# microsoft/XPretrain

Measured on NVIDIA H100. Metric: video-text pairs/sec (12f x 224^2, 32 tok), CLIP-ViP ViT-B/16 fwd+InfoNCE+bwd, higher is better.
Workload: dtype bf16

## Files before the change

### xpretrain_b200/csrc/gemm.cu

```cuda
#include "../../include/xpretrain_b200.h"
#include "common.h"
#include "ptx.cuh"
#include <cstdlib>

namespace xp {

constexpr int BM = 128;
constexpr int BK = 64;
constexpr int MMA_K = 16;
constexpr int GEMM_THREADS = 384;

struct GemmDev {
  void* c;
  const float* bias;
  const __nv_bfloat16* residual;
  __nv_bfloat16* aux;
  int M, N, K;
  long long ldc, ldr, ld_aux;
  long long c_group, c_group_stride, r_group, r_group_stride;
  int act;
  int splits;
  int scale_cols;
  float alpha, col_scale;
  uint32_t mn_lbo, mn_sbo;
};

template <int BN>
struct GemmCfg {
  static constexpr int A_BYTES = BM * BK * 2;
  static constexpr int B_BYTES = BN * BK * 2;
  static constexpr int STAGE_BYTES = A_BYTES + B_BYTES;
  static constexpr int STAGES = (BN == 256) ? 4 : 6;
  static constexpr int SMEM_BYTES = STAGES * STAGE_BYTES + 1024 + 256;
};

__device__ __forceinline__ float act_gelu_erf(float x) { return 0.5f * x * (1.f + erff(x * 0.70710678118654752f)); }
__device__ __forceinline__ float act_gelu_erf_grad(float x) {
  float cdf = 0.5f * (1.f + erff(x * 0.70710678118654752f));
  float pdf = 0.3989422804014327f * __expf(-0.5f * x * x);
  return cdf + x * pdf;
}

template <int BN, int A_MN, int B_MN, int OUT, int ACT>
__global__ void __launch_bounds__(GEMM_THREADS, 1)
gemm_kernel(const __grid_constant__ CUtensorMap tmA, const __grid_constant__ CUtensorMap tmB, const GemmDev p) {
  using Cfg = GemmCfg<BN>;
  constexpr int STAGES = Cfg::STAGES;
  constexpr bool PINGPONG = BN == 128;
  constexpr int MH = PINGPONG ? 2 : 1;
  constexpr int NH = BN / 128;
  extern __shared__ uint8_t smem_raw[];
  const uint32_t raw_addr = smem_u32(smem_raw);
  uint8_t* smem = smem_raw + (((raw_addr + 1023u) & ~1023u) - raw_addr);
  uint64_t* full_bar = reinterpret_cast<uint64_t*>(smem + STAGES * Cfg::STAGE_BYTES);
  uint64_t* empty_bar = full_bar + STAGES;

  const int wg = threadIdx.x >> 7;
  const int lane = threadIdx.x & 31;

  const int num_m = (p.M + BM - 1) / BM;
  const int num_n = (p.N + BN - 1) / BN;
  const int num_mn = num_m * num_n;
  const int total = num_mn * p.splits;
  const int kb_total = (p.K + BK - 1) / BK;
  const int kb_per = (kb_total + p.splits - 1) / p.splits;

  if (threadIdx.x == 0) {
    tma_prefetch_desc(&tmA);
    tma_prefetch_desc(&tmB);
    for (int s = 0; s < STAGES; ++s) {
      mbar_init(&full_bar[s], 1);
      mbar_init(&empty_bar[s], PINGPONG ? 1 : 2);
    }
    fence_barrier_init();
  }
  __syncthreads();

  if (wg == 0) {
    setmaxnreg_dec<40>();
    if (threadIdx.x == 0) {
      int stage = 0;
      uint32_t phase = 0;
      for (int tile = blockIdx.x; tile < total; tile += gridDim.x) {
        const int split = tile / num_mn;
        const int mn = tile - split * num_mn;
        const int m_blk = mn / num_n;
        const int n_blk = mn - m_blk * num_n;
        const int k0 = split * kb_per;
        const int k1 = min(kb_total, k0 + kb_per);
        for (int kb = k0; kb < k1; ++kb) {
          mbar_wait_nocall(&empty_bar[stage], phase ^ 1);
          uint8_t* sA = smem + stage * Cfg::STAGE_BYTES;
          uint8_t* sB = sA + Cfg::A_BYTES;
          mbar_arrive_expect_tx(&full_bar[stage], Cfg::STAGE_BYTES);
          if (A_MN) {
#pragma unroll
            for (int i = 0; i < BM / 64; ++i)
              tma_load_2d(sA + i * (BK * 128), &tmA, &full_bar[stage], m_blk * BM + i * 64, kb * BK);
          } else {
            tma_load_2d(sA, &tmA, &full_bar[stage], kb * BK, m_blk * BM);
          }
          if (B_MN) {
#pragma unroll
            for (int i = 0; i < BN / 64; ++i)
              tma_load_2d(sB + i * (BK * 128), &tmB, &full_bar[stage], n_blk * BN + i * 64, kb * BK);
          } else {
            tma_load_2d(sB, &tmB, &full_bar[stage], kb * BK, n_blk * BN);
          }
          if (++stage == STAGES) {
            stage = 0;
            phase ^= 1;
          }
        }
      }
    }
  } else {
    setmaxnreg_inc<232>();
    const int cw = wg - 1;
    const int wq = (threadIdx.x >> 5) & 3;
    constexpr int act = ACT;
    const int N = p.N, scale_cols = p.scale_cols;
    const float alpha = p.alpha, col_scale = p.col_scale;
    __nv_bfloat16* const aux_p = p.aux;
    constexpr bool need_aux_in = (ACT == XP_ACT_DQUICK_GELU || ACT == XP_ACT_DGELU_ERF);
    const __nv_bfloat16* const xin_p = need_aux_in ? p.aux : p.residual;
    constexpr uint32_t A_OFF = 64 * 128;
    const int cta_tiles = (total - blockIdx.x + gridDim.x - 1) / gridDim.x;
    int stage = 0;
    uint32_t phase = 0;
    int local = 0;
    for (int tile = blockIdx.x; tile < total; tile += gridDim.x, ++local) {
      const int split = tile / num_mn;
      const int mn = tile - split * num_mn;
      const int m_blk = mn / num_n;
      const int n_blk = mn - m_blk * num_n;
      const int k0 = split * kb_per;
      const int k1 = min(kb_total, k0 + kb_per);
      if (PINGPONG && (local & 1) != cw) {
        const int next = stage + max(0, k1 - k0);
        phase ^= (next / STAGES) & 1;
        stage = next % STAGES;
        continue;
      }
      if (PINGPONG && local > 0) named_bar_sync(1 + cw, 256);
      const bool pass_turn = PINGPONG && local + 1 < cta_tiles;
      if (k0 >= k1) {
        if (pass_turn) named_bar_arrive(2 - cw, 256);
        continue;
      }
      float acc[MH * NH][64];
#pragma unroll
      for (int q = 0; q < MH * NH; ++q)
#pragma unroll
        for (int i = 0; i < 64; ++i) acc[q][i] = 0.f;
      int prev_stage = -1;
      for (int kb = k0; kb < k1; ++kb) {
        mbar_wait_nocall(&full_bar[stage], phase);
        const uint32_t sA = smem_u32(smem + stage * Cfg::STAGE_BYTES) + (PINGPONG ? 0 : cw * A_OFF);
        const uint32_t sB = smem_u32(smem + stage * Cfg::STAGE_BYTES) + Cfg::A_BYTES;
#pragma unroll
        for (int q = 0; q < MH * NH; ++q) wgmma_fence_regs(acc[q]);
        wgmma_fence();
#pragma unroll
        for (int j = 0; j < BK / MMA_K; ++j) {
#pragma unroll
          for (int mh = 0; mh < MH; ++mh) {
            const uint32_t am = sA + mh * A_OFF;
            const uint64_t adesc = A_MN ? make_smem_desc_sw128(am + j * (MMA_K * 128), p.mn_lbo, p.mn_sbo)
                                        : make_smem_desc_sw128(am + j * (MMA_K * 2), 16, 1024);
#pragma unroll
            for (int h = 0; h < NH; ++h) {
              const uint32_t bh = sB + h * (128 * 128);
              const uint64_t bdesc = B_MN ? make_smem_desc_sw128(bh + j * (MMA_K * 128), p.mn_lbo, p.mn_sbo)
                                          : make_smem_desc_sw128(bh + j * (MMA_K * 2), 16, 1024);
              wgmma_m64n128k16_bf16<A_MN, B_MN>(acc[mh * NH + h], adesc, bdesc);
            }
          }
        }
        wgmma_commit();
#pragma unroll
        for (int q = 0; q < MH * NH; ++q) wgmma_fence_regs(acc[q]);
        wgmma_wait<1>();
        if (prev_stage >= 0 && (threadIdx.x & 127) == 0) mbar_arrive(&empty_bar[prev_stage]);
        prev_stage = stage;
        if (++stage == STAGES) {
          stage = 0;
          phase ^= 1;
        }
      }
      if (pass_turn) named_bar_arrive(2 - cw, 256);
      const auto load_bias = [&](float2(&b)[16], int h) {
#pragma unroll
        for (int i = 0; i < 16; ++i) {
          const int n = n_blk * BN + h * 128 + i * 8 + (lane & 3) * 2;
          b[i] = make_float2(0.f, 0.f);
          if (p.bias != nullptr && split == 0 && n < N) b[i] = __ldg(reinterpret_cast<const float2*>(p.bias + n));
        }
      };
      constexpr bool bias_once = PINGPONG && !need_aux_in;
      float2 bias_tile[16];
      if (bias_once) load_bias(bias_tile, 0);
      wgmma_wait<0>();
#pragma unroll
      for (int q = 0; q < MH * NH; ++q) wgmma_fence_regs(acc[q]);
      if ((threadIdx.x & 127) == 0) mbar_arrive(&empty_bar[prev_stage]);

      const auto apply = [&](float& v0, float& v1, int n, uint32_t xg) -> uint32_t {
        if (n < scale_cols) {
          v0 *= col_scale;
          v1 *= col_scale;
        }
        uint32_t pre = 0;
        if (act == XP_ACT_QUICK_GELU) {
          pre = pack_bf16(v0, v1);
          v0 = quick_gelu(v0);
          v1 = quick_gelu(v1);
        } else if (act == XP_ACT_DQUICK_GELU) {
          v0 *= quick_gelu_grad(bf16_lo(xg));
          v1 *= quick_gelu_grad(bf16_hi(xg));
        } else if (act == XP_ACT_GELU_ERF) {
          pre = pack_bf16(v0, v1);
          v0 = act_gelu_erf(v0);
          v1 = act_gelu_erf(v1);
        } else if (act == XP_ACT_DGELU_ERF) {
          v0 *= act_gelu_erf_grad(bf16_lo(xg));
          v1 *= act_gelu_erf_grad(bf16_hi(xg));
        } else if (xin_p != nullptr) {
          v0 += bf16_lo(xg);
          v1 += bf16_hi(xg);
        }
        return pre;
      };
      constexpr bool save_pre = (ACT == XP_ACT_QUICK_GELU || ACT == XP_ACT_GELU_ERF);
      const int quad = lane & 3;
#pragma unroll
      for (int mh = 0; mh < MH; ++mh) {
        const int row_base = m_blk * BM + (PINGPONG ? mh : cw) * 64 + wq * 16 + (lane >> 2);
#pragma unroll
        for (int rr = 0; rr < 2; ++rr) {
          const int row = row_base + rr * 8;
          const bool row_ok = row < p.M;
          const long long c_off = p.c_group > 0 ? (row / p.c_group) * p.c_group_stride + (row % p.c_group) * p.ldc
                                                : static_cast<long long>(row) * p.ldc;
          const long long x_off = need_aux_in ? static_cast<long long>(row) * p.ld_aux
                                              : (p.r_group > 0 ? (row / p.r_group) * p.r_group_stride + (row % p.r_group) * p.ldr
                                                               : static_cast<long long>(row) * p.ldr);
          const long long a_off = static_cast<long long>(row) * p.ld_aux;
#pragma unroll
          for (int h = 0; h < NH; ++h) {
            const float* const a = acc[mh * NH + h];
            const int n_h = n_blk * BN + h * 128;
            float2 bias2[16];
            if (bias_once) {
#pragma unroll
              for (int i = 0; i < 16; ++i) bias2[i] = bias_tile[i];
            } else {
              load_bias(bias2, h);
            }
            if (OUT == XP_OUT_BF16) {
              uint32_t xin[4][4];
#pragma unroll
              for (int k = 0; k < 4; ++k) {
                const int n8 = n_h + (4 * k + quad) * 8;
                uint4 v = make_uint4(0u, 0u, 0u, 0u);
                if (xin_p != nullptr && row_ok && n8 < N) v = *reinterpret_cast<const uint4*>(xin_p + x_off + n8);
                xin[k][0] = v.x;
                xin[k][1] = v.y;
                xin[k][2] = v.z;
                xin[k][3] = v.w;
                if (xin_p != nullptr) quad_transpose(xin[k]);
              }
#pragma unroll
              for (int k = 0; k < 4; ++k) {
                uint32_t out[4], pre[4];
#pragma unroll
                for (int j = 0; j < 4; ++j) {
                  const int i = 4 * k + j;
                  float v0 = fmaf(a[4 * i + 2 * rr], alpha, bias2[i].x);
                  float v1 = fmaf(a[4 * i + 2 * rr + 1], alpha, bias2[i].y);
                  pre[j] = apply(v0, v1, n_h + i * 8 + quad * 2, xin[k][j]);
                  out[j] = pack_bf16(v0, v1);
                }
                const int n8 = n_h + (4 * k + quad) * 8;
                quad_transpose(out);
                if (row_ok && n8 < N)
                  *reinterpret_cast<uint4*>(static_cast<__nv_bfloat16*>(p.c) + c_off + n8) =
                      make_uint4(out[0], out[1], out[2], out[3]);
                if (save_pre && aux_p != nullptr) {
                  quad_transpose(pre);
                  if (row_ok && n8 < N)
                    *reinterpret_cast<uint4*>(aux_p + a_off + n8) = make_uint4(pre[0], pre[1], pre[2], pre[3]);
                }
              }
            } else if (row_ok) {
              uint32_t xin[16];
#pragma unroll
              for (int i = 0; i < 16; ++i) {
                const int n = n_h + i * 8 + quad * 2;
                xin[i] = 0;
                if (xin_p != nullptr && n < N) xin[i] = *reinterpret_cast<const uint32_t*>(xin_p + x_off + n);
              }
#pragma unroll
              for (int i = 0; i < 16; ++i) {
                const int n = n_h + i * 8 + quad * 2;
                if (n >= N) continue;
                float v0 = fmaf(a[4 * i + 2 * rr], alpha, bias2[i].x);
                float v1 = fmaf(a[4 * i + 2 * rr + 1], alpha, bias2[i].y);
                apply(v0, v1, n, xin[i]);
                if (OUT == XP_OUT_F32) {
                  *reinterpret_cast<float2*>(static_cast<float*>(p.c) + c_off + n) = make_float2(v0, v1);
                } else {
                  asm volatile("red.global.add.v2.f32 [%0], {%1, %2};" ::"l"(static_cast<float*>(p.c) + c_off + n),
                               "f"(v0), "f"(v1)
                               : "memory");
                }
              }
            }
          }
        }
      }
    }
  }
}

template <int BN, int A_MN, int B_MN, int OUT, int ACT>
static int launch_gemm(const CUtensorMap& tmA, const CUtensorMap& tmB, const GemmDev& dev, int grid, cudaStream_t stream) {
  using Cfg = GemmCfg<BN>;
  auto kern = gemm_kernel<BN, A_MN, B_MN, OUT, ACT>;
  static bool attr_set = false;
  if (!attr_set) {
    XP_CHECK_CUDA(cudaFuncSetAttribute(kern, cudaFuncAttributeMaxDynamicSharedMemorySize, Cfg::SMEM_BYTES));
    attr_set = true;
  }
  kern<<<grid, GEMM_THREADS, Cfg::SMEM_BYTES, stream>>>(tmA, tmB, dev);
  XP_CHECK_LAUNCH("gemm_kernel");
  return 0;
}

template <int BN, int OUT, int ACT>
static int dispatch_layout(const XpGemm* g, const CUtensorMap& tmA, const CUtensorMap& tmB, const GemmDev& dev,
                           int grid, cudaStream_t stream) {
  if (g->a_layout == 0 && g->b_layout == 0) return launch_gemm<BN, 0, 0, OUT, ACT>(tmA, tmB, dev, grid, stream);
  if (g->a_layout == 0 && g->b_layout == 1) return launch_gemm<BN, 0, 1, OUT, ACT>(tmA, tmB, dev, grid, stream);
  if (g->a_layout == 1 && g->b_layout == 1) return launch_gemm<BN, 1, 1, OUT, ACT>(tmA, tmB, dev, grid, stream);
  if (g->a_layout == 1 && g->b_layout == 0) return launch_gemm<BN, 1, 0, OUT, ACT>(tmA, tmB, dev, grid, stream);
  return fail("xp_gemm: a_layout/b_layout must be 0 or 1");
}

template <int BN>
static int dispatch_act_bf16(const XpGemm* g, const CUtensorMap& tmA, const CUtensorMap& tmB, const GemmDev& dev, int grid,
                             cudaStream_t stream) {
  switch (g->act) {
    case XP_ACT_NONE: return dispatch_layout<BN, XP_OUT_BF16, XP_ACT_NONE>(g, tmA, tmB, dev, grid, stream);
    case XP_ACT_QUICK_GELU: return dispatch_layout<BN, XP_OUT_BF16, XP_ACT_QUICK_GELU>(g, tmA, tmB, dev, grid, stream);
    case XP_ACT_DQUICK_GELU: return dispatch_layout<BN, XP_OUT_BF16, XP_ACT_DQUICK_GELU>(g, tmA, tmB, dev, grid, stream);
    case XP_ACT_GELU_ERF: return dispatch_layout<BN, XP_OUT_BF16, XP_ACT_GELU_ERF>(g, tmA, tmB, dev, grid, stream);
    case XP_ACT_DGELU_ERF: return dispatch_layout<BN, XP_OUT_BF16, XP_ACT_DGELU_ERF>(g, tmA, tmB, dev, grid, stream);
  }
  return fail("xp_gemm: bad act");
}

template <int BN>
static int dispatch_out(const XpGemm* g, const CUtensorMap& tmA, const CUtensorMap& tmB, const GemmDev& dev, int grid,
                        cudaStream_t stream) {
  switch (g->out) {
    case XP_OUT_BF16: return dispatch_act_bf16<BN>(g, tmA, tmB, dev, grid, stream);
    case XP_OUT_F32: return dispatch_layout<BN, XP_OUT_F32, XP_ACT_NONE>(g, tmA, tmB, dev, grid, stream);
    case XP_OUT_F32_ATOMIC: return dispatch_layout<BN, XP_OUT_F32_ATOMIC, XP_ACT_NONE>(g, tmA, tmB, dev, grid, stream);
  }
  return fail("xp_gemm: bad out mode");
}

static int g_dbg_mn_lbo = 0, g_dbg_mn_sbo = 0;
}

extern "C" void xp_debug_gemm_mn_desc(int lbo, int sbo) {
  xp::g_dbg_mn_lbo = lbo;
  xp::g_dbg_mn_sbo = sbo;
}

extern "C" int xp_gemm(const XpGemm* g, void* stream_v) {
  using namespace xp;
  if (!g) return fail("xp_gemm: null args");
  cudaStream_t stream = static_cast<cudaStream_t>(stream_v);
  if (g->M <= 0 || g->N <= 0 || g->K <= 0) return fail("xp_gemm: M, N, K must be positive");
  if (g->N % 8 != 0) return fail("xp_gemm: N must be a multiple of 8");
  if (!g->a || !g->b || !g->c) return fail("xp_gemm: null operand");
  XP_ENTER(g->a);
  const int splits = g->splits <= 0 ? 1 : g->splits;
  if (splits > 1 && g->out != XP_OUT_F32_ATOMIC) return fail("xp_gemm: split-K requires XP_OUT_F32_ATOMIC");
  if ((g->act == XP_ACT_DQUICK_GELU || g->act == XP_ACT_DGELU_ERF) && !g->aux)
    return fail("xp_gemm: dGELU epilogue needs aux (the forward pre-activation)");
  if (g->act != XP_ACT_NONE && g->out != XP_OUT_BF16) return fail("xp_gemm: activation epilogues need a bf16 output");
  if (g->act != XP_ACT_NONE && g->residual)
    return fail("xp_gemm: a residual add cannot be combined with an activation epilogue");
  if (g->aux && g->c_group > 0) return fail("xp_gemm: aux cannot be combined with grouped rows (c_group > 0)");
  if (g->scale_cols < 0 || g->scale_cols % 2) return fail("xp_gemm: scale_cols must be even and non-negative");
  const int elem_c = g->out == XP_OUT_BF16 ? 2 : 4;
  if ((reinterpret_cast<uintptr_t>(g->c) & 15) || (g->ldc * elem_c) % 16)
    return fail("xp_gemm: C must be 16-byte aligned with a 16-byte multiple row pitch");
  if (g->bias && (reinterpret_cast<uintptr_t>(g->bias) & 15)) return fail("xp_gemm: bias must be 16-byte aligned");
  if (g->residual && ((reinterpret_cast<uintptr_t>(g->residual) & 15) || (g->ldr % 8)))
    return fail("xp_gemm: residual must be 16-byte aligned, ldr % 8 == 0");
  if (g->aux && ((reinterpret_cast<uintptr_t>(g->aux) & 15) || (g->ld_aux % 8)))
    return fail("xp_gemm: aux must be 16-byte aligned, ld_aux % 8 == 0");
  if ((g->c_group > 0 && g->c_group_stride % 8) || (g->r_group > 0 && g->r_group_stride % 8))
    return fail("xp_gemm: c_group_stride / r_group_stride must be multiples of 8 elements");

  const int nsm = sm_count();
  const int num_m = static_cast<int>((g->M + BM - 1) / BM);
  int bn = g->block_n;
  if (bn == 0) {
    const long long tiles256 = static_cast<long long>(num_m) * ((g->N + 255) / 256) * splits;
    const long long kb_split = ((g->K + BK - 1) / BK + splits - 1) / splits;
    const bool short_k_fwd = g->b_layout == 0 && kb_split <= 16;
    bn = (g->N >= 256 && tiles256 >= nsm && !short_k_fwd) ? 256 : 128;
  }
  if (bn != 128 && bn != 256) return fail("xp_gemm: block_n must be 0, 128 or 256");
  if (g->cta_pair < 0 || g->cta_pair > 1) return fail("xp_gemm: cta_pair must be 0 or 1 (no CTA pairs on sm_90)");
  const long long total = static_cast<long long>(num_m) * ((g->N + bn - 1) / bn) * splits;
  int grid = g->max_ctas > 0 ? g->max_ctas : nsm;
  if (grid < 1) grid = 1;
  if (grid > total) grid = static_cast<int>(total);

  CUtensorMap tmA, tmB;
  int rc;
  if (g->a_layout == 0)
    rc = make_tmap_bf16_2d(&tmA, g->a, g->K, g->M, g->lda, BK, BM);
  else
    rc = make_tmap_bf16_2d(&tmA, g->a, g->M, g->K, g->lda, 64, BK);
  if (rc) return rc;
  if (g->b_layout == 0)
    rc = make_tmap_bf16_2d(&tmB, g->b, g->K, g->N, g->ldb, BK, bn);
  else
    rc = make_tmap_bf16_2d(&tmB, g->b, g->N, g->K, g->ldb, 64, BK);
  if (rc) return rc;

  GemmDev dev;
  dev.c = g->c;
  dev.bias = g->bias;
  dev.residual = static_cast<const __nv_bfloat16*>(g->residual);
  dev.aux = static_cast<__nv_bfloat16*>(g->aux);
  dev.M = static_cast<int>(g->M);
  dev.N = static_cast<int>(g->N);
  dev.K = static_cast<int>(g->K);
  dev.ldc = g->ldc;
  dev.ldr = g->ldr;
  dev.ld_aux = g->ld_aux;
  dev.c_group = g->c_group;
  dev.c_group_stride = g->c_group_stride;
  dev.r_group = g->r_group;
  dev.r_group_stride = g->r_group_stride;
  dev.act = g->act;
  dev.splits = splits;
  dev.scale_cols = g->scale_cols;
  dev.alpha = g->alpha;
  dev.col_scale = g->col_scale;
  dev.mn_lbo = g_dbg_mn_lbo ? g_dbg_mn_lbo : BK * 128;
  dev.mn_sbo = g_dbg_mn_sbo ? g_dbg_mn_sbo : 1024;

  return bn == 256 ? dispatch_out<256>(g, tmA, tmB, dev, grid, stream)
                   : dispatch_out<128>(g, tmA, tmB, dev, grid, stream);
}
```

### xpretrain_b200/csrc/ptx.cuh

```cuda
#pragma once
#include <cuda.h>
#include <cuda_bf16.h>
#include <cuda_runtime.h>
#include <stdint.h>
#include <stdio.h>

namespace xp {

#ifndef XP_WAIT_TIMEOUT_CYCLES
#define XP_WAIT_TIMEOUT_CYCLES (8000000000ll)
#endif

__device__ __forceinline__ uint32_t smem_u32(const void* p) {
  return static_cast<uint32_t>(__cvta_generic_to_shared(p));
}
__device__ __forceinline__ int lane_id() { return threadIdx.x & 31; }

__device__ __forceinline__ void mbar_init(uint64_t* bar, uint32_t count) {
  asm volatile("mbarrier.init.shared::cta.b64 [%0], %1;" ::"r"(smem_u32(bar)), "r"(count) : "memory");
}
__device__ __forceinline__ void fence_barrier_init() {
  asm volatile("fence.mbarrier_init.release.cluster;" ::: "memory");
}
__device__ __forceinline__ void fence_proxy_async_smem() {
  asm volatile("fence.proxy.async.shared::cta;" ::: "memory");
}
__device__ __forceinline__ void mbar_arrive_expect_tx(uint64_t* bar, uint32_t bytes) {
  asm volatile("mbarrier.arrive.expect_tx.shared::cta.b64 _, [%0], %1;" ::"r"(smem_u32(bar)), "r"(bytes)
               : "memory");
}
__device__ __forceinline__ void mbar_arrive(uint64_t* bar) {
  asm volatile("mbarrier.arrive.shared::cta.b64 _, [%0];" ::"r"(smem_u32(bar)) : "memory");
}
__device__ __forceinline__ bool mbar_try_wait(uint64_t* bar, uint32_t parity) {
  uint32_t ok;
  asm volatile(
      "{\n"
      ".reg .pred p;\n"
      "mbarrier.try_wait.parity.shared::cta.b64 p, [%1], %2;\n"
      "selp.u32 %0, 1, 0, p;\n"
      "}\n"
      : "=r"(ok)
      : "r"(smem_u32(bar)), "r"(parity)
      : "memory");
  return ok != 0;
}
__device__ __forceinline__ void mbar_wait(uint64_t* bar, uint32_t parity) {
  if (mbar_try_wait(bar, parity)) return;
  long long t0 = clock64();
  while (!mbar_try_wait(bar, parity)) {
    if (clock64() - t0 > XP_WAIT_TIMEOUT_CYCLES) {
      printf("xpretrain_b200: mbarrier wait timeout (block %d thread %d parity %u)\n", blockIdx.x, threadIdx.x,
             parity);
      __trap();
    }
  }
}
__device__ __forceinline__ void mbar_wait_nocall(uint64_t* bar, uint32_t parity) {
  if (mbar_try_wait(bar, parity)) return;
  long long t0 = clock64();
  while (!mbar_try_wait(bar, parity)) {
    if (clock64() - t0 > XP_WAIT_TIMEOUT_CYCLES) __trap();
  }
}

__device__ __forceinline__ void tma_prefetch_desc(const CUtensorMap* m) {
  asm volatile("prefetch.tensormap [%0];" ::"l"(reinterpret_cast<uint64_t>(m)) : "memory");
}
__device__ __forceinline__ void tma_load_2d(void* smem_dst, const CUtensorMap* m, uint64_t* bar, int c0, int c1) {
  asm volatile(
      "cp.async.bulk.tensor.2d.shared::cluster.global.mbarrier::complete_tx::bytes [%0], [%1, {%3, %4}], [%2];"
      ::"r"(smem_u32(smem_dst)), "l"(reinterpret_cast<uint64_t>(m)), "r"(smem_u32(bar)), "r"(c0), "r"(c1)
      : "memory");
}
__device__ __forceinline__ void tma_load_3d(void* smem_dst, const CUtensorMap* m, uint64_t* bar, int c0, int c1,
                                            int c2) {
  asm volatile(
      "cp.async.bulk.tensor.3d.shared::cluster.global.mbarrier::complete_tx::bytes [%0], [%1, {%3, %4, %5}], [%2];"
      ::"r"(smem_u32(smem_dst)), "l"(reinterpret_cast<uint64_t>(m)), "r"(smem_u32(bar)), "r"(c0), "r"(c1), "r"(c2)
      : "memory");
}

__device__ __forceinline__ void tma_store_2d(const CUtensorMap* m, uint32_t smem_src, int c0, int c1) {
  asm volatile("cp.async.bulk.tensor.2d.global.shared::cta.bulk_group [%0, {%2, %3}], [%1];" ::"l"(
                   reinterpret_cast<uint64_t>(m)),
               "r"(smem_src), "r"(c0), "r"(c1)
               : "memory");
}
__device__ __forceinline__ void tma_store_commit() { asm volatile("cp.async.bulk.commit_group;" ::: "memory"); }
template <int N>
__device__ __forceinline__ void tma_store_wait_read() {
  asm volatile("cp.async.bulk.wait_group.read %0;" ::"n"(N) : "memory");
}

__device__ __forceinline__ void wgmma_fence() { asm volatile("wgmma.fence.sync.aligned;" ::: "memory"); }
__device__ __forceinline__ void wgmma_commit() { asm volatile("wgmma.commit_group.sync.aligned;" ::: "memory"); }
template <int N>
__device__ __forceinline__ void wgmma_wait() {
  asm volatile("wgmma.wait_group.sync.aligned %0;" ::"n"(N) : "memory");
}
template <int R>
__device__ __forceinline__ void wgmma_fence_regs(float (&d)[R]) {
#pragma unroll
  for (int i = 0; i < R; ++i) asm volatile("" : "+f"(d[i])::"memory");
}

template <int TA, int TB>
__device__ __forceinline__ void wgmma_m64n128k16_bf16(float (&d)[64], uint64_t adesc, uint64_t bdesc) {
  asm volatile(
      "wgmma.mma_async.sync.aligned.m64n128k16.f32.bf16.bf16 {"
      "%0, %1, %2, %3, %4, %5, %6, %7, %8, %9, %10, %11, %12, %13, %14, %15, "
      "%16, %17, %18, %19, %20, %21, %22, %23, %24, %25, %26, %27, %28, %29, %30, %31, "
      "%32, %33, %34, %35, %36, %37, %38, %39, %40, %41, %42, %43, %44, %45, %46, %47, "
      "%48, %49, %50, %51, %52, %53, %54, %55, %56, %57, %58, %59, %60, %61, %62, %63"
      "}, %64, %65, 1, 1, 1, %66, %67;"
      : "+f"(d[0]), "+f"(d[1]), "+f"(d[2]), "+f"(d[3]), "+f"(d[4]), "+f"(d[5]), "+f"(d[6]), "+f"(d[7]),
        "+f"(d[8]), "+f"(d[9]), "+f"(d[10]), "+f"(d[11]), "+f"(d[12]), "+f"(d[13]), "+f"(d[14]), "+f"(d[15]),
        "+f"(d[16]), "+f"(d[17]), "+f"(d[18]), "+f"(d[19]), "+f"(d[20]), "+f"(d[21]), "+f"(d[22]), "+f"(d[23]),
        "+f"(d[24]), "+f"(d[25]), "+f"(d[26]), "+f"(d[27]), "+f"(d[28]), "+f"(d[29]), "+f"(d[30]), "+f"(d[31]),
        "+f"(d[32]), "+f"(d[33]), "+f"(d[34]), "+f"(d[35]), "+f"(d[36]), "+f"(d[37]), "+f"(d[38]), "+f"(d[39]),
        "+f"(d[40]), "+f"(d[41]), "+f"(d[42]), "+f"(d[43]), "+f"(d[44]), "+f"(d[45]), "+f"(d[46]), "+f"(d[47]),
        "+f"(d[48]), "+f"(d[49]), "+f"(d[50]), "+f"(d[51]), "+f"(d[52]), "+f"(d[53]), "+f"(d[54]), "+f"(d[55]),
        "+f"(d[56]), "+f"(d[57]), "+f"(d[58]), "+f"(d[59]), "+f"(d[60]), "+f"(d[61]), "+f"(d[62]), "+f"(d[63])
      : "l"(adesc), "l"(bdesc), "n"(TA), "n"(TB));
}

template <int TA, int TB>
__device__ __forceinline__ void wgmma_m64n64k16_ss(float (&d)[32], uint64_t adesc, uint64_t bdesc) {
  asm volatile(
      "wgmma.mma_async.sync.aligned.m64n64k16.f32.bf16.bf16 {"
      "%0, %1, %2, %3, %4, %5, %6, %7, %8, %9, %10, %11, %12, %13, %14, %15, "
      "%16, %17, %18, %19, %20, %21, %22, %23, %24, %25, %26, %27, %28, %29, %30, %31"
      "}, %32, %33, 1, 1, 1, %34, %35;"
      : "+f"(d[0]), "+f"(d[1]), "+f"(d[2]), "+f"(d[3]), "+f"(d[4]), "+f"(d[5]), "+f"(d[6]), "+f"(d[7]),
        "+f"(d[8]), "+f"(d[9]), "+f"(d[10]), "+f"(d[11]), "+f"(d[12]), "+f"(d[13]), "+f"(d[14]), "+f"(d[15]),
        "+f"(d[16]), "+f"(d[17]), "+f"(d[18]), "+f"(d[19]), "+f"(d[20]), "+f"(d[21]), "+f"(d[22]), "+f"(d[23]),
        "+f"(d[24]), "+f"(d[25]), "+f"(d[26]), "+f"(d[27]), "+f"(d[28]), "+f"(d[29]), "+f"(d[30]), "+f"(d[31])
      : "l"(adesc), "l"(bdesc), "n"(TA), "n"(TB));
}
template <int TB>
__device__ __forceinline__ void wgmma_m64n64k16_rs(float (&d)[32], const uint32_t (&a)[4], uint64_t bdesc) {
  asm volatile(
      "wgmma.mma_async.sync.aligned.m64n64k16.f32.bf16.bf16 {"
      "%0, %1, %2, %3, %4, %5, %6, %7, %8, %9, %10, %11, %12, %13, %14, %15, "
      "%16, %17, %18, %19, %20, %21, %22, %23, %24, %25, %26, %27, %28, %29, %30, %31"
      "}, {%32, %33, %34, %35}, %36, 1, 1, 1, %37;"
      : "+f"(d[0]), "+f"(d[1]), "+f"(d[2]), "+f"(d[3]), "+f"(d[4]), "+f"(d[5]), "+f"(d[6]), "+f"(d[7]),
        "+f"(d[8]), "+f"(d[9]), "+f"(d[10]), "+f"(d[11]), "+f"(d[12]), "+f"(d[13]), "+f"(d[14]), "+f"(d[15]),
        "+f"(d[16]), "+f"(d[17]), "+f"(d[18]), "+f"(d[19]), "+f"(d[20]), "+f"(d[21]), "+f"(d[22]), "+f"(d[23]),
        "+f"(d[24]), "+f"(d[25]), "+f"(d[26]), "+f"(d[27]), "+f"(d[28]), "+f"(d[29]), "+f"(d[30]), "+f"(d[31])
      : "r"(a[0]), "r"(a[1]), "r"(a[2]), "r"(a[3]), "l"(bdesc), "n"(TB));
}

template <uint32_t N>
__device__ __forceinline__ void setmaxnreg_dec() {
  asm volatile("setmaxnreg.dec.sync.aligned.u32 %0;" ::"n"(N));
}
template <uint32_t N>
__device__ __forceinline__ void setmaxnreg_inc() {
  asm volatile("setmaxnreg.inc.sync.aligned.u32 %0;" ::"n"(N));
}
__device__ __forceinline__ void named_bar_sync(uint32_t id, uint32_t threads) {
  asm volatile("bar.sync %0, %1;" ::"r"(id), "r"(threads) : "memory");
}
__device__ __forceinline__ void named_bar_arrive(uint32_t id, uint32_t threads) {
  asm volatile("bar.arrive %0, %1;" ::"r"(id), "r"(threads) : "memory");
}

__device__ __forceinline__ uint64_t make_smem_desc_sw128(uint32_t smem_addr, uint32_t lbo_bytes,
                                                         uint32_t sbo_bytes) {
  uint64_t d = 0;
  d |= static_cast<uint64_t>((smem_addr & 0x3FFFF) >> 4);
  d |= static_cast<uint64_t>((lbo_bytes >> 4) & 0x3FFF) << 16;
  d |= static_cast<uint64_t>((sbo_bytes >> 4) & 0x3FFF) << 32;
  d |= static_cast<uint64_t>(1) << 62;
  return d;
}

__device__ __forceinline__ void quad_transpose(uint32_t (&v)[4]) {
  const int q = threadIdx.x & 3;
  uint32_t out[4];
  out[0] = out[1] = out[2] = out[3] = 0u;
#pragma unroll
  for (int t = 0; t < 4; ++t) {
    const int j = q ^ t;
    const uint32_t send = j == 0 ? v[0] : j == 1 ? v[1] : j == 2 ? v[2] : v[3];
    const uint32_t got = t == 0 ? send : __shfl_xor_sync(0xffffffffu, send, t);
#pragma unroll
    for (int c = 0; c < 4; ++c)
      if (c == j) out[c] = got;
  }
#pragma unroll
  for (int c = 0; c < 4; ++c) v[c] = out[c];
}

__device__ __forceinline__ uint32_t pack_bf16(float lo, float hi) {
  __nv_bfloat162 v = __floats2bfloat162_rn(lo, hi);
  return *reinterpret_cast<uint32_t*>(&v);
}
__device__ __forceinline__ float bf16_lo(uint32_t v) { return __uint_as_float(v << 16); }
__device__ __forceinline__ float bf16_hi(uint32_t v) { return __uint_as_float(v & 0xFFFF0000u); }

__device__ __forceinline__ float fast_sigmoid(float y) {
  float t;
  asm("tanh.approx.f32 %0, %1;" : "=f"(t) : "f"(0.5f * y));
  return fmaf(0.5f, t, 0.5f);
}
__device__ __forceinline__ float quick_gelu(float x) { return x * fast_sigmoid(1.702f * x); }
__device__ __forceinline__ float quick_gelu_grad(float x) {
  float y = 1.702f * x;
  y = y > 64.f ? 64.f : (y < -64.f ? -64.f : y);
  const float s = fast_sigmoid(y);
  return s * fmaf(y, 1.f - s, 1.f);
}

}
```

Measured before the change: 291.6.

## Stage bf16 GEMM epilogue in swizzled smem and write via TMA stores

For BN=128 ping-pong bf16 GEMMs, each consumer warpgroup now writes its output tile into swizzled shared-memory slots and issues TMA 2D stores instead of per-thread global stores. For dGELU backward it also prefetches the saved pre-activation tile into shared memory via TMA ahead of the epilogue, and it tracks aliasing between input and output. Pipeline stages drop from 6 to 5 to make room for staging buffers. The BN=256 heuristic now treats short-K problems as short regardless of B layout. This adds barrier and store-wait synchronisation and fewer mainloop stages.

```diff
diff --git a/xpretrain_b200/csrc/gemm.cu b/xpretrain_b200/csrc/gemm.cu
--- a/xpretrain_b200/csrc/gemm.cu
+++ b/xpretrain_b200/csrc/gemm.cu
@@ -2,6 +2,7 @@
 #include "common.h"
 #include "ptx.cuh"
 #include <cstdlib>
+#include <cstring>
 
 namespace xp {
 
@@ -23,15 +24,19 @@
   int scale_cols;
   float alpha, col_scale;
   uint32_t mn_lbo, mn_sbo;
+  int xin_alias;
 };
 
-template <int BN>
+template <int BN, bool TMA_OUT>
 struct GemmCfg {
   static constexpr int A_BYTES = BM * BK * 2;
   static constexpr int B_BYTES = BN * BK * 2;
   static constexpr int STAGE_BYTES = A_BYTES + B_BYTES;
-  static constexpr int STAGES = (BN == 256) ? 4 : 6;
-  static constexpr int SMEM_BYTES = STAGES * STAGE_BYTES + 1024 + 256;
+  static constexpr int SLOT_BYTES = 64 * 128 * 2;
+  static constexpr int STAGING_BYTES = TMA_OUT ? 2 * 2 * SLOT_BYTES : 0;
+  static constexpr int STAGES = (BN == 256) ? 4 : (TMA_OUT ? 5 : 6);
+  static constexpr int SMEM_BYTES = STAGES * STAGE_BYTES + STAGING_BYTES + 1024 + 256;
+  static_assert(SMEM_BYTES <= 227 * 1024, "shared memory per block on sm_90");
 };
 
 __device__ __forceinline__ float act_gelu_erf(float x) { return 0.5f * x * (1.f + erff(x * 0.70710678118654752f)); }
@@ -41,10 +46,12 @@
   return cdf + x * pdf;
 }
 
-template <int BN, int A_MN, int B_MN, int OUT, int ACT>
+template <int BN, int A_MN, int B_MN, int OUT, int ACT, bool TMA_OUT>
 __global__ void __launch_bounds__(GEMM_THREADS, 1)
-gemm_kernel(const __grid_constant__ CUtensorMap tmA, const __grid_constant__ CUtensorMap tmB, const GemmDev p) {
-  using Cfg = GemmCfg<BN>;
+gemm_kernel(const __grid_constant__ CUtensorMap tmA, const __grid_constant__ CUtensorMap tmB,
+            const __grid_constant__ CUtensorMap tmC, const __grid_constant__ CUtensorMap tmX, const GemmDev p) {
+  using Cfg = GemmCfg<BN, TMA_OUT>;
+  static_assert(!TMA_OUT || (BN == 128 && OUT == XP_OUT_BF16), "TMA-stored outputs: ping-pong bf16 tiles only");
   constexpr int STAGES = Cfg::STAGES;
   constexpr bool PINGPONG = BN == 128;
   constexpr int MH = PINGPONG ? 2 : 1;
@@ -52,8 +59,9 @@
   extern __shared__ uint8_t smem_raw[];
   const uint32_t raw_addr = smem_u32(smem_raw);
   uint8_t* smem = smem_raw + (((raw_addr + 1023u) & ~1023u) - raw_addr);
-  uint64_t* full_bar = reinterpret_cast<uint64_t*>(smem + STAGES * Cfg::STAGE_BYTES);
+  uint64_t* full_bar = reinterpret_cast<uint64_t*>(smem + STAGES * Cfg::STAGE_BYTES + Cfg::STAGING_BYTES);
   uint64_t* empty_bar = full_bar + STAGES;
+  uint64_t* pre_bar = empty_bar + STAGES;
 
   const int wg = threadIdx.x >> 7;
   const int lane = threadIdx.x & 31;
@@ -68,6 +76,12 @@
   if (threadIdx.x == 0) {
     tma_prefetch_desc(&tmA);
     tma_prefetch_desc(&tmB);
+    if (TMA_OUT) {
+      tma_prefetch_desc(&tmC);
+      if (ACT != XP_ACT_NONE && p.aux != nullptr) tma_prefetch_desc(&tmX);
+      mbar_init(&pre_bar[0], 1);
+      mbar_init(&pre_bar[1], 1);
+    }
     for (int s = 0; s < STAGES; ++s) {
       mbar_init(&full_bar[s], 1);
       mbar_init(&empty_bar[s], PINGPONG ? 1 : 2);
@@ -126,6 +140,28 @@
     const __nv_bfloat16* const xin_p = need_aux_in ? p.aux : p.residual;
     constexpr uint32_t A_OFF = 64 * 128;
     const int cta_tiles = (total - blockIdx.x + gridDim.x - 1) / gridDim.x;
+    constexpr bool pre_in_smem = TMA_OUT && need_aux_in;
+    const uint32_t slots = smem_u32(smem) + STAGES * Cfg::STAGE_BYTES + cw * 2 * Cfg::SLOT_BYTES;
+    const bool leader = (threadIdx.x & 127) == 0;
+    uint32_t pre_phase = 0;
+    const auto prefetch_pre = [&](int t) {
+      const int mb = t / num_n, nb = t - mb * num_n;
+      uint32_t bytes = 0;
+#pragma unroll
+      for (int mh = 0; mh < 2; ++mh)
+#pragma unroll
+        for (int b = 0; b < 2; ++b)
+          if (mb * BM + mh * 64 < p.M && nb * BN + b * 64 < N) bytes += 64 * 128;
+      mbar_arrive_expect_tx(&pre_bar[cw], bytes);
+#pragma unroll
+      for (int mh = 0; mh < 2; ++mh)
+#pragma unroll
+        for (int b = 0; b < 2; ++b)
+          if (mb * BM + mh * 64 < p.M && nb * BN + b * 64 < N)
+            tma_load_2d(smem + STAGES * Cfg::STAGE_BYTES + (cw * 2 + mh) * Cfg::SLOT_BYTES + b * (64 * 128), &tmX,
+                        &pre_bar[cw], nb * BN + b * 64, mb * BM + mh * 64);
+    };
+    if (pre_in_smem && leader && cw < cta_tiles) prefetch_pre(blockIdx.x + cw * gridDim.x);
     int stage = 0;
     uint32_t phase = 0;
     int local = 0;
@@ -233,9 +269,27 @@
       };
       constexpr bool save_pre = (ACT == XP_ACT_QUICK_GELU || ACT == XP_ACT_GELU_ERF);
       const int quad = lane & 3;
+      const bool two_out = save_pre && aux_p != nullptr;
+      if (pre_in_smem) {
+        mbar_wait_nocall(&pre_bar[cw], pre_phase);
+        pre_phase ^= 1;
+      } else if (TMA_OUT && xin_p != nullptr && p.xin_alias) {
+        if (leader) tma_store_wait<0>();
+        named_bar_sync(3 + cw, 128);
+      }
 #pragma unroll
       for (int mh = 0; mh < MH; ++mh) {
         const int row_base = m_blk * BM + (PINGPONG ? mh : cw) * 64 + wq * 16 + (lane >> 2);
+        if (TMA_OUT && !pre_in_smem) {
+          if (leader) {
+            if (two_out)
+              tma_store_wait_read<0>();
+            else
+              tma_store_wait_read<1>();
+          }
+          named_bar_sync(3 + cw, 128);
+        }
+        const uint32_t out_slot = slots + (two_out ? 0 : mh) * Cfg::SLOT_BYTES;
 #pragma unroll
         for (int rr = 0; rr < 2; ++rr) {
           const int row = row_base + rr * 8;
@@ -263,23 +317,39 @@
               for (int k = 0; k < 4; ++k) {
                 const int n8 = n_h + (4 * k + quad) * 8;
                 uint4 v = make_uint4(0u, 0u, 0u, 0u);
-                if (xin_p != nullptr && row_ok && n8 < N) v = *reinterpret_cast<const uint4*>(xin_p + x_off + n8);
+                if (!pre_in_smem && xin_p != nullptr && row_ok && n8 < N)
+                  v = *reinterpret_cast<const uint4*>(xin_p + x_off + n8);
                 xin[k][0] = v.x;
                 xin[k][1] = v.y;
                 xin[k][2] = v.z;
                 xin[k][3] = v.w;
-                if (xin_p != nullptr) quad_transpose(xin[k]);
+                if (!pre_in_smem && xin_p != nullptr) quad_transpose(xin[k]);
               }
 #pragma unroll
               for (int k = 0; k < 4; ++k) {
                 uint32_t out[4], pre[4];
+                const uint32_t row_addr = out_slot + (wq * 16 + rr * 8 + (lane >> 2)) * 128 + quad * 4;
+                const auto slot_addr = [&](int i) -> uint32_t {
+                  return row_addr + (i >> 3) * (64 * 128) + (((i & 7) << 4) ^ ((lane >> 2) << 4));
+                };
 #pragma unroll
                 for (int j = 0; j < 4; ++j) {
                   const int i = 4 * k + j;
                   float v0 = fmaf(a[4 * i + 2 * rr], alpha, bias2[i].x);
                   float v1 = fmaf(a[4 * i + 2 * rr + 1], alpha, bias2[i].y);
-                  pre[j] = apply(v0, v1, n_h + i * 8 + quad * 2, xin[k][j]);
+                  const uint32_t xg = pre_in_smem ? ld_shared_u32(slot_addr(i)) : xin[k][j];
+                  pre[j] = apply(v0, v1, n_h + i * 8 + quad * 2, xg);
                   out[j] = pack_bf16(v0, v1);
+                }
+                if (TMA_OUT) {
+#pragma unroll
+                  for (int j = 0; j < 4; ++j) {
+                    const int i = 4 * k + j;
+                    const uint32_t addr = slot_addr(i);
+                    st_shared_u32(addr, out[j]);
+                    if (two_out) st_shared_u32(addr + Cfg::SLOT_BYTES, pre[j]);
+                  }
+                  continue;
                 }
                 const int n8 = n_h + (4 * k + quad) * 8;
                 quad_transpose(out);
@@ -318,66 +388,109 @@
             }
           }
         }
+        if (TMA_OUT) {
+          fence_proxy_async_smem();
+          named_bar_sync(3 + cw, 128);
+          const int row0 = m_blk * BM + mh * 64;
+          if (leader && row0 < p.M) {
+#pragma unroll
+            for (int b = 0; b < 2; ++b) {
+              const int col = n_blk * BN + b * 64;
+              if (col >= N) continue;
+              tma_store_2d(&tmC, out_slot + b * (64 * 128), col, row0);
+              if (two_out) tma_store_2d(&tmX, out_slot + Cfg::SLOT_BYTES + b * (64 * 128), col, row0);
+            }
+          }
+          if (leader) tma_store_commit();
+          if (leader && mh == MH - 1 && local + 2 >= cta_tiles) tma_store_wait<0>();
+          if (pre_in_smem && leader && mh == MH - 1 && local + 2 < cta_tiles) {
+            if (p.xin_alias)
+              tma_store_wait<0>();
+            else
+              tma_store_wait_read<0>();
+            prefetch_pre(tile + 2 * gridDim.x);
+          }
+        }
       }
     }
   }
 }
 
-template <int BN, int A_MN, int B_MN, int OUT, int ACT>
-static int launch_gemm(const CUtensorMap& tmA, const CUtensorMap& tmB, const GemmDev& dev, int grid, cudaStream_t stream) {
-  using Cfg = GemmCfg<BN>;
-  auto kern = gemm_kernel<BN, A_MN, B_MN, OUT, ACT>;
+template <int BN, int A_MN, int B_MN, int OUT, int ACT, bool TMA_OUT>
+static int launch_gemm(const CUtensorMap& tmA, const CUtensorMap& tmB, const CUtensorMap& tmC, const CUtensorMap& tmX,
+                       const GemmDev& dev, int grid, cudaStream_t stream) {
+  using Cfg = GemmCfg<BN, TMA_OUT>;
+  auto kern = gemm_kernel<BN, A_MN, B_MN, OUT, ACT, TMA_OUT>;
   static bool attr_set = false;
   if (!attr_set) {
     XP_CHECK_CUDA(cudaFuncSetAttribute(kern, cudaFuncAttributeMaxDynamicSharedMemorySize, Cfg::SMEM_BYTES));
     attr_set = true;
   }
-  kern<<<grid, GEMM_THREADS, Cfg::SMEM_BYTES, stream>>>(tmA, tmB, dev);
+  kern<<<grid, GEMM_THREADS, Cfg::SMEM_BYTES, stream>>>(tmA, tmB, tmC, tmX, dev);
   XP_CHECK_LAUNCH("gemm_kernel");
   return 0;
 }
 
-template <int BN, int OUT, int ACT>
-static int dispatch_layout(const XpGemm* g, const CUtensorMap& tmA, const CUtensorMap& tmB, const GemmDev& dev,
-                           int grid, cudaStream_t stream) {
-  if (g->a_layout == 0 && g->b_layout == 0) return launch_gemm<BN, 0, 0, OUT, ACT>(tmA, tmB, dev, grid, stream);
-  if (g->a_layout == 0 && g->b_layout == 1) return launch_gemm<BN, 0, 1, OUT, ACT>(tmA, tmB, dev, grid, stream);
-  if (g->a_layout == 1 && g->b_layout == 1) return launch_gemm<BN, 1, 1, OUT, ACT>(tmA, tmB, dev, grid, stream);
-  if (g->a_layout == 1 && g->b_layout == 0) return launch_gemm<BN, 1, 0, OUT, ACT>(tmA, tmB, dev, grid, stream);
+struct GemmMaps {
+  CUtensorMap a, b, c, x;
+};
+
+template <int BN, int OUT, int ACT, bool TMA_OUT>
+static int dispatch_layout(const XpGemm* g, const GemmMaps& m, const GemmDev& dev, int grid, cudaStream_t stream) {
+  if (g->a_layout == 0 && g->b_layout == 0)
+    return launch_gemm<BN, 0, 0, OUT, ACT, TMA_OUT>(m.a, m.b, m.c, m.x, dev, grid, stream);
+  if (g->a_layout == 0 && g->b_layout == 1)
+    return launch_gemm<BN, 0, 1, OUT, ACT, TMA_OUT>(m.a, m.b, m.c, m.x, dev, grid, stream);
+  if (g->a_layout == 1 && g->b_layout == 1)
+    return launch_gemm<BN, 1, 1, OUT, ACT, TMA_OUT>(m.a, m.b, m.c, m.x, dev, grid, stream);
+  if (g->a_layout == 1 && g->b_layout == 0)
+    return launch_gemm<BN, 1, 0, OUT, ACT, TMA_OUT>(m.a, m.b, m.c, m.x, dev, grid, stream);
   return fail("xp_gemm: a_layout/b_layout must be 0 or 1");
 }
 
+template <int BN, bool TMA_OUT>
+static int dispatch_act_bf16(const XpGemm* g, const GemmMaps& m, const GemmDev& dev, int grid, cudaStream_t stream) {
+  switch (g->act) {
+    case XP_ACT_NONE: return dispatch_layout<BN, XP_OUT_BF16, XP_ACT_NONE, TMA_OUT>(g, m, dev, grid, stream);
+    case XP_ACT_QUICK_GELU: return dispatch_layout<BN, XP_OUT_BF16, XP_ACT_QUICK_GELU, TMA_OUT>(g, m, dev, grid, stream);
+    case XP_ACT_DQUICK_GELU: return dispatch_layout<BN, XP_OUT_BF16, XP_ACT_DQUICK_GELU, TMA_OUT>(g, m, dev, grid, stream);
+    case XP_ACT_GELU_ERF: return dispatch_layout<BN, XP_OUT_BF16, XP_ACT_GELU_ERF, TMA_OUT>(g, m, dev, grid, stream);
+    case XP_ACT_DGELU_ERF: return dispatch_layout<BN, XP_OUT_BF16, XP_ACT_DGELU_ERF, TMA_OUT>(g, m, dev, grid, stream);
+  }
+  return fail("xp_gemm: bad act");
+}
+
 template <int BN>
-static int dispatch_act_bf16(const XpGemm* g, const CUtensorMap& tmA, const CUtensorMap& tmB, const GemmDev& dev, int grid,
-                             cudaStream_t stream) {
-  switch (g->act) {
-    case XP_ACT_NONE: return dispatch_layout<BN, XP_OUT_BF16, XP_ACT_NONE>(g, tmA, tmB, dev, grid, stream);
-    case XP_ACT_QUICK_GELU: return dispatch_layout<BN, XP_OUT_BF16, XP_ACT_QUICK_GELU>(g, tmA, tmB, dev, grid, stream);
-    case XP_ACT_DQUICK_GELU: return dispatch_layout<BN, XP_OUT_BF16, XP_ACT_DQUICK_GELU>(g, tmA, tmB, dev, grid, stream);
-    case XP_ACT_GELU_ERF: return dispatch_layout<BN, XP_OUT_BF16, XP_ACT_GELU_ERF>(g, tmA, tmB, dev, grid, stream);
-    case XP_ACT_DGELU_ERF: return dispatch_layout<BN, XP_OUT_BF16, XP_ACT_DGELU_ERF>(g, tmA, tmB, dev, grid, stream);
-  }
-  return fail("xp_gemm: bad act");
-}
-
-template <int BN>
-static int dispatch_out(const XpGemm* g, const CUtensorMap& tmA, const CUtensorMap& tmB, const GemmDev& dev, int grid,
-                        cudaStream_t stream) {
+static int dispatch_out(const XpGemm* g, const GemmMaps& m, const GemmDev& dev, int grid, cudaStream_t stream,
+                        bool tma_out) {
   switch (g->out) {
-    case XP_OUT_BF16: return dispatch_act_bf16<BN>(g, tmA, tmB, dev, grid, stream);
-    case XP_OUT_F32: return dispatch_layout<BN, XP_OUT_F32, XP_ACT_NONE>(g, tmA, tmB, dev, grid, stream);
-    case XP_OUT_F32_ATOMIC: return dispatch_layout<BN, XP_OUT_F32_ATOMIC, XP_ACT_NONE>(g, tmA, tmB, dev, grid, stream);
+    case XP_OUT_BF16:
+      if constexpr (BN == 128) {
+        if (tma_out) return dispatch_act_bf16<BN, true>(g, m, dev, grid, stream);
+      }
+      return dispatch_act_bf16<BN, false>(g, m, dev, grid, stream);
+    case XP_OUT_F32: return dispatch_layout<BN, XP_OUT_F32, XP_ACT_NONE, false>(g, m, dev, grid, stream);
+    case XP_OUT_F32_ATOMIC: return dispatch_layout<BN, XP_OUT_F32_ATOMIC, XP_ACT_NONE, false>(g, m, dev, grid, stream);
   }
   return fail("xp_gemm: bad out mode");
 }
 
 static int g_dbg_mn_lbo = 0, g_dbg_mn_sbo = 0;
+static bool g_dbg_register_epilogue = false;
+
+static bool bf16_rows_overlap(const void* a, long long lda, const void* b, long long ldb, long long M, long long N) {
+  const uintptr_t lo_a = reinterpret_cast<uintptr_t>(a), lo_b = reinterpret_cast<uintptr_t>(b);
+  const uintptr_t hi_a = lo_a + static_cast<uintptr_t>(((M - 1) * lda + N) * 2);
+  const uintptr_t hi_b = lo_b + static_cast<uintptr_t>(((M - 1) * ldb + N) * 2);
+  return lo_a < hi_b && lo_b < hi_a;
+}
 }
 
 extern "C" void xp_debug_gemm_mn_desc(int lbo, int sbo) {
   xp::g_dbg_mn_lbo = lbo;
   xp::g_dbg_mn_sbo = sbo;
 }
+extern "C" void xp_debug_gemm_register_epilogue(int on) { xp::g_dbg_register_epilogue = on != 0; }
 
 extern "C" int xp_gemm(const XpGemm* g, void* stream_v) {
   using namespace xp;
@@ -413,8 +526,8 @@
   if (bn == 0) {
     const long long tiles256 = static_cast<long long>(num_m) * ((g->N + 255) / 256) * splits;
     const long long kb_split = ((g->K + BK - 1) / BK + splits - 1) / splits;
-    const bool short_k_fwd = g->b_layout == 0 && kb_split <= 16;
-    bn = (g->N >= 256 && tiles256 >= nsm && !short_k_fwd) ? 256 : 128;
+    const bool short_k = kb_split <= 16;
+    bn = (g->N >= 256 && tiles256 >= nsm && !short_k) ? 256 : 128;
   }
   if (bn != 128 && bn != 256) return fail("xp_gemm: block_n must be 0, 128 or 256");
   if (g->cta_pair < 0 || g->cta_pair > 1) return fail("xp_gemm: cta_pair must be 0 or 1 (no CTA pairs on sm_90)");
@@ -423,18 +536,26 @@
   if (grid < 1) grid = 1;
   if (grid > total) grid = static_cast<int>(total);
 
-  CUtensorMap tmA, tmB;
+  GemmMaps maps;
+  memset(&maps, 0, sizeof(maps));
   int rc;
   if (g->a_layout == 0)
-    rc = make_tmap_bf16_2d(&tmA, g->a, g->K, g->M, g->lda, BK, BM);
+    rc = make_tmap_bf16_2d(&maps.a, g->a, g->K, g->M, g->lda, BK, BM);
   else
-    rc = make_tmap_bf16_2d(&tmA, g->a, g->M, g->K, g->lda, 64, BK);
+    rc = make_tmap_bf16_2d(&maps.a, g->a, g->M, g->K, g->lda, 64, BK);
   if (rc) return rc;
   if (g->b_layout == 0)
-    rc = make_tmap_bf16_2d(&tmB, g->b, g->K, g->N, g->ldb, BK, bn);
+    rc = make_tmap_bf16_2d(&maps.b, g->b, g->K, g->N, g->ldb, BK, bn);
   else
-    rc = make_tmap_bf16_2d(&tmB, g->b, g->N, g->K, g->ldb, 64, BK);
+    rc = make_tmap_bf16_2d(&maps.b, g->b, g->N, g->K, g->ldb, 64, BK);
   if (rc) return rc;
+  const bool dgelu = g->act == XP_ACT_DQUICK_GELU || g->act == XP_ACT_DGELU_ERF;
+  const bool tma_out = bn == 128 && g->out == XP_OUT_BF16 && g->c_group == 0 && !g_dbg_register_epilogue;
+  const bool save_pre = g->act == XP_ACT_QUICK_GELU || g->act == XP_ACT_GELU_ERF;
+  if (tma_out) {
+    if ((rc = make_tmap_bf16_2d(&maps.c, g->c, g->N, g->M, g->ldc, 64, 64))) return rc;
+    if ((save_pre || dgelu) && (rc = make_tmap_bf16_2d(&maps.x, g->aux, g->N, g->M, g->ld_aux, 64, 64))) return rc;
+  }
 
   GemmDev dev;
   dev.c = g->c;
@@ -458,7 +579,12 @@
   dev.col_scale = g->col_scale;
   dev.mn_lbo = g_dbg_mn_lbo ? g_dbg_mn_lbo : BK * 128;
   dev.mn_sbo = g_dbg_mn_sbo ? g_dbg_mn_sbo : 1024;
-
-  return bn == 256 ? dispatch_out<256>(g, tmA, tmB, dev, grid, stream)
-                   : dispatch_out<128>(g, tmA, tmB, dev, grid, stream);
-}
+  dev.xin_alias = 0;
+  if (tma_out && dgelu)
+    dev.xin_alias = bf16_rows_overlap(g->aux, g->ld_aux, g->c, g->ldc, g->M, g->N);
+  else if (tma_out && g->residual)
+    dev.xin_alias = g->r_group > 0 || bf16_rows_overlap(g->residual, g->ldr, g->c, g->ldc, g->M, g->N);
+
+  return bn == 256 ? dispatch_out<256>(g, maps, dev, grid, stream, false)
+                   : dispatch_out<128>(g, maps, dev, grid, stream, tma_out);
+}
diff --git a/xpretrain_b200/csrc/ptx.cuh b/xpretrain_b200/csrc/ptx.cuh
--- a/xpretrain_b200/csrc/ptx.cuh
+++ b/xpretrain_b200/csrc/ptx.cuh
@@ -15,6 +15,14 @@
   return static_cast<uint32_t>(__cvta_generic_to_shared(p));
 }
 __device__ __forceinline__ int lane_id() { return threadIdx.x & 31; }
+__device__ __forceinline__ uint32_t ld_shared_u32(uint32_t addr) {
+  uint32_t v;
+  asm volatile("ld.shared.b32 %0, [%1];" : "=r"(v) : "r"(addr) : "memory");
+  return v;
+}
+__device__ __forceinline__ void st_shared_u32(uint32_t addr, uint32_t v) {
+  asm volatile("st.shared.b32 [%0], %1;" ::"r"(addr), "r"(v) : "memory");
+}
 
 __device__ __forceinline__ void mbar_init(uint64_t* bar, uint32_t count) {
   asm volatile("mbarrier.init.shared::cta.b64 [%0], %1;" ::"r"(smem_u32(bar)), "r"(count) : "memory");
@@ -91,6 +99,10 @@
 template <int N>
 __device__ __forceinline__ void tma_store_wait_read() {
   asm volatile("cp.async.bulk.wait_group.read %0;" ::"n"(N) : "memory");
+}
+template <int N>
+__device__ __forceinline__ void tma_store_wait() {
+  asm volatile("cp.async.bulk.wait_group %0;" ::"n"(N) : "memory");
 }
 
 __device__ __forceinline__ void wgmma_fence() { asm volatile("wgmma.fence.sync.aligned;" ::: "memory"); }
```

New measurement: 310.8, median of 6. 6.6% higher.
